# ehsan886/DBA_mod

Hardware: AMD Instinct MI355X
Metric: FL rounds/sec + backdoor ASR & main-task acc, ResNet-18 CIFAR-10 100 clients (higher is better)
Workload: dtype fp32

## Files before the change

### csrc/kernels/xconv_fwd.hip

```cpp
#include "xhalo.hpp"

namespace xg {
SplitPolicy& split_policy() {
  static SplitPolicy p;
  return p;
}
int& xstage_mode() {
  static int mode = 1;
  return mode;
}
XLast& last_launch() {
  static XLast l{};
  return l;
}
}

namespace {

template <int W, int IMGS, int BN, int WM, int WN, bool PRE>
__global__ __launch_bounds__(256) void ximg_kernel(const XArgs a) {
  constexpr int P = 2, NT = 256;
  constexpr int PW = W + 2, PI = PW * PW, PP = IMGS * PI;
  constexpr int CC = 32, CH = CC / 8, Q4 = CC / 4;
  constexpr int PATCH = PP * CH;
// ... 231 lines not shown
    split4h(pv[u].x, pv[u].y, pv[u].z, pv[u].w, hs.ma, sp);
    const int o = pp * CH + ((q >> 1) ^ (prow & 3));
#pragma unroll
    for (int p = 0; p < P; ++p) ((uint2*)&ximg2_patch[(buf * P + p) * PATCH + o])[q & 1] = sp[p];
  };

  const __amdgpu_buffer_rsrc_t rF = rsrc(a.wf + (long long)slot * a.wf_sstride, (long long)a.Ncol * 9 * Cs * 4);
  const int wbase = ((n0 >> 5) + wn) * NK * 4096 + lane * 16;
  uint4 wb[3][4];
  auto gw = [&](int t, int s, int f) __attribute__((always_inline)) {
    wb[s][f] = __builtin_bit_cast(uint4, bload4(rF, t < NK ? wbase + t * 4096 + f * 1024 : kOOB));
  };

  f32x16_t acc[MI][1];
#pragma unroll
  for (int i = 0; i < MI; ++i)
#pragma unroll
    for (int r = 0; r < 16; ++r) acc[i][0][r] = 0.f;

  int apix[MI], arow[MI];
#pragma unroll
  for (int i = 0; i < MI; ++i) {
    const int m = wm * TM + i * 32 + fr;
    const int im = m / (W * W), rem = m - im * (W * W);
    apix[i] = im * PI + (rem / W) * PW + rem % W;
    arow[i] = rem / W;
  }

  hs.init(amax_read(a.amax_src, a.amax_src_ld, g), amax_read(a.amax_w, a.amax_w_ld, slot));
#pragma unroll
  for (int f = 0; f < 4; ++f) {
    gw(0, 0, f);
    gw(1, 1, f);
  }
#pragma unroll
  for (int u = 0; u < NE; ++u) pload1(u, 0);
#pragma unroll
  for (int u = 0; u < NE; ++u) {
    ppiece(u, 0);
    pload1(u, 1);
  }
  __syncthreads();
  for (int c = 0; c < NC; ++c) {
    const uint4* L = ximg2_patch + (c & 1) * P * PATCH;
    const bool more = c + 1 < NC;
    sfor<9>([&](auto TAP) __attribute__((always_inline)) {
      constexpr int tap = decltype(TAP)::value, ti = tap / 3, tj = tap - ti * 3;
      constexpr int toff = ti * PW + tj, s = tap % 3, s2 = (tap + 2) % 3;
      constexpr int u = tap - (9 - NE);
      constexpr int NQ = u >= 0 ? 5 : 4;
      const int t = c * 9 + tap;
      __builtin_amdgcn_sched_barrier(0x786);
      sfor<2>([&](auto KK) __attribute__((always_inline)) {
        constexpr int kk = decltype(KK)::value;
        const int ch = kk * 2 + hf;
        uint4 af[P][MI], bfr[P][1];
#pragma unroll
        for (int i = 0; i < MI; ++i) {
          const int o = (apix[i] + toff) * CH + (ch ^ ((arow[i] + ti) & 3));
#pragma unroll
          for (int p = 0; p < P; ++p) af[p][i] = L[p * PATCH + o];
        }
#pragma unroll
        for (int p = 0; p < P; ++p) bfr[p][0] = wb[s][kk * 2 + p];
        mma_half<MI, 1, P, true, NQ, kk>(af, bfr, acc, [&](int q) __attribute__((always_inline)) {
          if (q < 4) {
            gw(t + 2, s2, q);
          } else if constexpr (u >= 0) {
            if (more) ppiece(u, (c + 1) & 1);
            pload1(u, c + 2);
          }
        });
      });
    });
    __syncthreads();
  }
  hs.finish(acc);

  float* out = a.out + (long long)g * a.out_gstride;
  const float* bias = a.bias ? a.bias + (long long)slot * a.b_sstride : nullptr;
  const float* res = a.res ? a.res + (long long)g * a.out_gstride : nullptr;
  float vmax = 0.f;
  const int n = n0 + wn * 32 + fr;
  if (n < a.Ncol) {
    const float bv = bias ? bias[n] : 0.f;
#pragma unroll
    for (int i = 0; i < MI; ++i)
#pragma unroll
      for (int r = 0; r < 16; ++r) {
        const int m = wm * TM + i * 32 + (r & 3) + 8 * (r >> 2) + 4 * hf;
        if (img0 + m / (W * W) >= nv) continue;
        const long long o = (long long)(img0 * W * W + m) * a.Ncol + n;
        float v = acc[i][0][r];
        if (bias) v += bv;
        if (res) v += res[o];
        if (a.relu) v = relu_nan(v);
        vmax = fmaxf(vmax, fabsf(v));
        out[o] = v;
      }
  }
  if (a.amax_out) amax_fold(a.amax_out, a.amax_out_ld, g, vmax);
}

template <int W, int IMGS, int BN, int WM, int WN>
int ximg_go(const XArgs& a, int G, hipStream_t st) {
  XArgs b = a;
  b.tiles_n = ceil_div(a.Ncol, BN);
  const dim3 grid((unsigned)(ceil_div(a.N, IMGS) * b.tiles_n), G, 1);
  xg::last_launch() = XLast{3, W, BN, a.wp != nullptr, 0, 1, 1, 0};
  if (a.wp) hipLaunchKernelGGL((ximg_kernel<W, IMGS, BN, WM, WN, true>), grid, dim3(256), 0, st, b);
  else hipLaunchKernelGGL((ximg_kernel<W, IMGS, BN, WM, WN, false>), grid, dim3(256), 0, st, b);
  DBA_LAUNCH_CHECK();
}
template <int W, int IMGS, int BN>
int ximg2_go(const XArgs& a, int G, hipStream_t st) {
  constexpr int PATCH = IMGS * (W + 2) * (W + 2) * 4;
  constexpr int LDS = 2 * 2 * PATCH * (int)sizeof(uint4);
  static unsigned long long attr_set = 0ull;
  int dev = 0;
  if (hipGetDevice(&dev) != hipSuccess || dev < 0 || dev >= 64) return -100;
  if (!(attr_set >> dev & 1ull)) {
    if (hipFuncSetAttribute((const void*)ximg2_kernel<W, IMGS, BN>, hipFuncAttributeMaxDynamicSharedMemorySize,
                            LDS) != hipSuccess)
      return -100;
    attr_set |= 1ull << dev;
  }
  XArgs b = a;
  b.tiles_n = ceil_div(a.Ncol, BN);
  const dim3 grid((unsigned)(ceil_div(a.N, IMGS) * b.tiles_n), G, 1);
  xg::last_launch() = XLast{4, W, BN, 1, 0, 1, 1, 0};
  hipLaunchKernelGGL((ximg2_kernel<W, IMGS, BN>), grid, dim3(256), LDS, st, b);
  DBA_LAUNCH_CHECK();
}
__global__ __launch_bounds__(256) void xstage16_kernel(const XArgs a) {
  constexpr int P = 2, W = 16, CS = 64, BM = 128, BN = 64, WN = 2;
  constexpr int TR = BM / W, PW = W + 2, PR = TR + 2, PP = PR * PW;
  constexpr int CH = CS / 8, PATCH = PP * CH;
  constexpr int TM = 64, TN = 32, MI = TM / 32;
  constexpr int CB = CS / 32;
  constexpr int STG = (BN / 32) * CB * 4 * 64;
  static_assert(BM * BN <= P * PATCH * 4, "epilogue tile fits the patch");
  __shared__ __attribute__((aligned(16))) uint4 lds[P * PATCH + 2 * STG];
  __shared__ long long orow[BM];
  uint4* const patch = lds;
  uint4* const bring = lds + P * PATCH;

  const int g = blockIdx.y;
  const int HT = a.Ho / TR;
  const int tm = blockIdx.x;
  const int img = tm / HT, h0 = (tm - img * HT) * TR;
  if (img >= valid_rows(a.nvalid, g, a.N)) return;
  const int slot = a.wsel ? a.wsel[g] : g;
  const float* __restrict__ src = a.src + (long long)g * a.src_gstride;
  const int tid = threadIdx.x, lane = tid & 63, wid = tid >> 6;
  const int wm = wid / WN, wn = wid % WN;
  const int fr = lane & 31, hf = lane >> 5;

  const uint16_t* F = a.wf + (long long)slot * a.wf_sstride + ((wid >> 1) * (CB * 9) + (wid & 1) * 9) * 2048 + lane * 8;
  auto fill = [&](int tap) __attribute__((always_inline)) {
    const uint32_t dst = __builtin_amdgcn_readfirstlane(
        (uint32_t)(uintptr_t)(__attribute__((address_space(3))) void*)(bring + (tap & 1) * STG + wid * 256));
#pragma unroll
    for (int f = 0; f < 4; ++f) {
      uint32_t keep;
      asm volatile("s_mov_b32 %0, m0\n\ts_mov_b32 m0, %2\n\ts_nop 0\n\tglobal_load_lds_dwordx4 %1, off\n\ts_mov_b32 m0, %0"
                   : "=&s"(keep)
                   : "v"(F + tap * 2048 + f * 512), "s"(dst + f * 1024)
                   : "memory");
    }
  };
  auto gl_sync = [&]() __attribute__((always_inline)) {
    asm volatile("s_waitcnt vmcnt(0)" ::: "memory");
    __syncthreads();
  };
  fill(0);

  if (tid < BM)
    orow[tid] = (((long long)img * a.Ho + h0 + tid / W) * a.Wo + tid % W) * a.Ncol;

  constexpr int Q4 = CS / 4;
  constexpr int NE = (PP * Q4 + 255) / 256;
  float4 pv[NE];
  {
    const __amdgpu_buffer_rsrc_t rA = rsrc(src, (long long)a.N * a.Hs * a.Ws * CS * 4);
#pragma unroll
    for (int u = 0; u < NE; ++u) {
      const int e = tid + 256 * u;
      const int pp = e / Q4, q = e - pp * Q4;
      const int pr = pp / PW, pc = pp - pr * PW;
      const int h = h0 - 1 + pr, w = pc - 1;
      const bool ok = e < PP * Q4 && (unsigned)h < (unsigned)a.Hs && (unsigned)w < (unsigned)a.Ws;
      pv[u] = bload4(rA, ok ? (((img * a.Hs + h) * a.Ws + w) * CS + q * 4) * 4 : kOOB);
    }
  }
  HScale hs;
  hs.init(amax_read(a.amax_src, a.amax_src_ld, g), amax_read(a.amax_w, a.amax_w_ld, slot));
#pragma unroll
  for (int u = 0; u < NE; ++u) {
    const int e = tid + 256 * u;
    if (e >= PP * Q4) break;
    const int pp = e / Q4, q = e - pp * Q4;
    uint2 sp[P];
    split4h(pv[u].x, pv[u].y, pv[u].z, pv[u].w, hs.ma, sp);
    const int o = pp * CH + ((q >> 1) ^ hswz<W, CS>(pp, pp % PW));
#pragma unroll
    for (int p = 0; p < P; ++p) ((uint2*)&patch[p * PATCH + o])[q & 1] = sp[p];
  }

  f32x16_t acc[MI][1];
#pragma unroll
  for (int i = 0; i < MI; ++i)
#pragma unroll
    for (int r = 0; r < 16; ++r) acc[i][0][r] = 0.f;
  int apix[MI], acol[MI];
#pragma unroll
  for (int i = 0; i < MI; ++i) {
    const int m = wm * TM + i * 32 + fr;
    apix[i] = (m / W) * PW + (m % W);
    acol[i] = m % W;
  }

  auto stage = [&](int tap) __attribute__((always_inline)) {
    const int ti = tap / 3, tj = tap - ti * 3;
    const int toff = ti * PW + tj;
    const uint4* L = bring + (tap & 1) * STG + wn * (CB * 4 * 64) + lane;
    uint4 af[2][P][MI], bfr[2][P][1];
    auto frags = [&](auto Hc) __attribute__((always_inline)) {
      constexpr int h = decltype(Hc)::value, cb = h / 2, kk = h % 2, st = h & 1;
      const int ch = kk * 2 + hf;
#pragma unroll
      for (int i = 0; i < MI; ++i) {
        const int pp = apix[i] + toff;
        const int o = pp * CH + ((cb * 4 + ch) ^ hswz<W, CS>(pp, acol[i] + tj));
#pragma unroll
        for (int p = 0; p < P; ++p) af[st][p][i] = patch[p * PATCH + o];
      }
#pragma unroll
      for (int p = 0; p < P; ++p) bfr[st][p][0] = L[(cb * 4 + kk * 2 + p) * 64];
    };
    frags(std::integral_constant<int, 0>{});
    sfor<2 * CB>([&](auto Hc) __attribute__((always_inline)) {
      constexpr int h = decltype(Hc)::value;
      if constexpr (h + 1 < 2 * CB) frags(std::integral_constant<int, h + 1>{});
      __builtin_amdgcn_sched_barrier(0);
      mma_half<MI, 1, P, true, 0, h % 2>(af[h & 1], bfr[h & 1], acc, [](int) {});
      __builtin_amdgcn_sched_barrier(0);
    });
  };

  gl_sync();
  for (int tap = 0; tap < 9; ++tap) {
    if (tap + 1 < 9) fill(tap + 1);
    stage(tap);
    gl_sync();
  }
  hs.finish(acc);

  float* Ct = reinterpret_cast<float*>(patch);
#pragma unroll
  for (int i = 0; i < MI; ++i)
#pragma unroll
    for (int r = 0; r < 16; ++r)
      Ct[(wm * TM + i * 32 + (r & 3) + 8 * (r >> 2) + 4 * hf) * BN + wn * TN + fr] = acc[i][0][r];
  __syncthreads();
  float* out = a.out + (long long)g * a.out_gstride;
  const float* bias = a.bias ? a.bias + (long long)slot * a.b_sstride : nullptr;
  const float* res = a.res ? a.res + (long long)g * a.out_gstride : nullptr;
  constexpr int C4 = BN / 4;
  float vmax = 0.f;
  for (int e = tid; e < BM * C4; e += 256) {
    const int row = e / C4, n = (e - row * C4) * 4;
    const long long o = orow[row];
    float4 v = *(const float4*)&Ct[row * BN + n];
    if (bias) { v.x += bias[n]; v.y += bias[n + 1]; v.z += bias[n + 2]; v.w += bias[n + 3]; }
    if (res) {
      const float4 rv = *(const float4*)(res + o + n);
      v.x += rv.x; v.y += rv.y; v.z += rv.z; v.w += rv.w;
    }
    if (a.relu) relu_nan4(v);
    vmax = fmaxf(vmax, fmaxf(fmaxf(fabsf(v.x), fabsf(v.y)), fmaxf(fabsf(v.z), fabsf(v.w))));
    *(float4*)(out + o + n) = v;
  }
  if (a.amax_out) amax_fold(a.amax_out, a.amax_out_ld, g, vmax);
}

constexpr bool kXStage16Default = true;

int xstage16_try(const XArgs& a, int G, int KH, int KW, hipStream_t st) {
  const XClass& c = a.cls[0];
  const int mode = xg::xstage_mode();
  if (!(mode == 3 || (mode == 1 && kXStage16Default))) return -100;
  if (KH != 3 || KW != 3 || a.sp != 1 || a.os != 1 || a.dsg != 1 || a.splitk != 1 || c.nI != 3 || c.nJ != 3 ||
      c.bh != -1 || c.bw != -1)
    return -100;
  if (a.Hs != 16 || a.Ws != 16 || a.Ho != 16 || a.Wo != 16 || a.Cs != 64 || a.Ncol != 64) return -100;
  if (a.bf.mode || a.lz_coef || a.sc_src) return -100;
  if (!aligned16(a.src) || !aligned16(a.w) || a.src_gstride % 4 || a.w_sstride % 4) return -100;
  if (!a.wp || !a.wf || ((uintptr_t)a.wf & 15) || a.wf_sstride % 8 || a.wf_sstride < 2 * 64 * 576) return -100;
  xg::last_launch() = XLast{5, 16, 64, 1, 0, 1, 1, 0};
  hipLaunchKernelGGL(xstage16_kernel, dim3((unsigned)(a.N * (a.Ho / 8)), G, 1), dim3(256), 0, st, a);
  DBA_LAUNCH_CHECK();
}

int& ximg_on() {
  static int on = 1;
  return on;
}
int ximg_try(const XArgs& a, int G, int KH, int KW, hipStream_t st) {
  const XClass& c = a.cls[0];
  if (!ximg_on() || KH != 3 || KW != 3 || a.sp != 1 || a.os != 1 || a.dsg != 1 || a.splitk != 1 || c.nI != 3 ||
      c.nJ != 3 || c.bh != -1 || c.bw != -1)
    return -100;
  if (a.Hs != a.Ho || a.Ws != a.Wo || a.Ho != a.Wo || a.Cs % 32 != 0 || a.Ncol % 32 != 0) return -100;
  if (a.bf.mode || a.lz_coef) return -100;
  if (!aligned16(a.src) || a.src_gstride % 4 || !aligned16(a.w) || a.w_sstride % 4) return -100;
  if (a.wp && (((uintptr_t)a.wp & 15) || a.wp_sstride % 8)) return -100;
  if (a.sc_src) return -100;
  if (ximg_on() == 1 && a.wp && a.wf && !((uintptr_t)a.wf & 15) && a.wf_sstride % 8 == 0) {
    int rc = -100;
    if (a.Wo == 8) rc = a.Ncol >= 128 ? ximg2_go<8, 2, 128>(a, G, st) : ximg2_go<8, 2, 64>(a, G, st);
    if (a.Wo == 4) rc = a.Ncol >= 128 ? ximg2_go<4, 8, 128>(a, G, st) : ximg2_go<4, 8, 64>(a, G, st);
    if (rc != -100) return rc;
  }
  if (a.Wo == 8) return a.Ncol >= 128 ? ximg_go<8, 2, 128, 2, 2>(a, G, st) : ximg_go<8, 2, 64, 2, 2>(a, G, st);
  if (a.Wo == 4) return a.Ncol >= 128 ? ximg_go<4, 8, 128, 2, 2>(a, G, st) : ximg_go<4, 8, 64, 2, 2>(a, G, st);
  return -100;
}

}

DBA_EXPORT int dba_xsplit_policy(int target, int min_k, int max_s, int kslab_max, int dgrad_ks) {
  SplitPolicy& p = split_policy();
  if (dgrad_ks >= 0) p.dgrad_ks = dgrad_ks;
  if (target > 0) p.target = target;
  if (min_k > 0) p.min_k = min_k;
  if (max_s > 0) p.max_s = std::min(max_s, kSkMax);
  if (kslab_max > 0) p.kslab_max = kslab_max;
  return 0;
}

DBA_EXPORT int dba_xconv_last_launch(int* out) {
  const XLast& l = xg::last_launch();
  const int v[8] = {l.kind, l.tile, l.vec, l.pre, l.form, l.slabs, l.nclass, l.lazy};
  for (int i = 0; i < 8; ++i) out[i] = v[i];
  return 0;
}

DBA_EXPORT int dba_ximg_set(int on) {
  const int prev = ximg_on();
  if (on >= 0) ximg_on() = on;
  return prev;
}

DBA_EXPORT int dba_xstage_set(int on) {
  const int prev = xg::xstage_mode();
  if (on >= 1 && on <= 3) xg::xstage_mode() = on;
  return prev;
}


DBA_EXPORT long long dba_xconv_ws_floats(int G, int N, int Ho, int Wo, int Cin, int Cout, int KH, int KW) {
  const long long M = (long long)N * Ho * Wo;
  const int s = xsplitk(M, G, Cout, KH * KW * Cin);
  return s > 1 ? (long long)s * G * M * Cout : 0;
}


DBA_EXPORT long long dba_xconv_sk_ints(int G, int N, int Ho, int Wo, int Cin, int Cout, int KH, int KW) {
  const long long M = (long long)N * Ho * Wo;
  const int s = xsplitk(M, G, Cout, KH * KW * Cin);
  const long long n = s > 1 ? xconv_sk_count(M, Cout, G, 1, s) : 0;
  return (n > 0 && sk_ok((const int*)1, n, M, Cout, G, 1, s)) ? n : 0;
}


DBA_EXPORT int dba_xconv_fwd(const float* x, long long x_gstride, const float* w, long long w_sstride,
                             const int* wsel, const float* bias, long long b_sstride, const float* res, float* out,
                             long long out_gstride, const int* nvalid, int G, int N, int H, int W, int Cin, int Ho,
                             int Wo, int Cout, int KH, int KW, int stride, int pad, int relu, const int* amax_x,
                             int amax_x_ld, const int* amax_w, int amax_w_ld, int* amax_out, int amax_out_ld,
                             const uint16_t* wp, long long wp_sstride, const uint16_t* wf, long long wf_sstride,
                             float* ws, long long ws_floats, int* sk_cnt,
                             long long sk_cnt_n, const void* bnf, const float* lz_coef, int lz_relu,
                             void* stream) {
  hipStream_t st = (hipStream_t)stream;
  if ((long long)N * H * W * Cin >= (1LL << 29)) return -103;
  const long long M = (long long)N * Ho * Wo;
  const int K = KH * KW * Cin;
  const int vec = (Cin % 4 == 0 && aligned16(x) && aligned16(w) && x_gstride % 4 == 0 && w_sstride % 4 == 0) ? 4 : 1;
  XArgs a{};
  a.src = x; a.src_gstride = x_gstride; a.w = w; a.w_sstride = w_sstride; a.wsel = wsel;
  a.bias = bias; a.b_sstride = b_sstride; a.res = res; a.out = out; a.out_gstride = out_gstride;
  a.nvalid = nvalid; a.N = N; a.Hs = H; a.Ws = W; a.Cs = Cin; a.Ncol = Cout; a.Ho = Ho; a.Wo = Wo;
  a.sp = stride; a.os = 1; a.dsg = 1; a.relu = relu; a.splitk = 1;
  a.amax_src = amax_x; a.amax_w = amax_w; a.amax_out = amax_out;
  a.amax_src_ld = amax_x_ld; a.amax_w_ld = amax_w_ld; a.amax_out_ld = amax_out_ld;
  a.wp = wp; a.wp_sstride = wp_sstride; a.wf = wf; a.wf_sstride = wf_sstride;
  a.cls[0] = XClass{KH, KW, -pad, -pad, 0, 0, Ho, Wo, 0};
  if (!amax_x || !amax_w) return -109;
  if (bnf) {
    a.bf = *(const BnFuse*)bnf;
    if (a.bf.mode != 1 || bias || res || relu || (Cout & 3) || a.bf.C != Cout) return -108;
  }
  if (lz_coef) {
    if (wp || vec < 4 || Cin > 512) return -108;
    a.lz_coef = lz_coef; a.lz_relu = lz_relu;
  }
  auto fin = [&](int rc) { return (rc == 0 && a.bf.mode) ? bnx_finalize_go(a.bf, nvalid, G, N, Ho * Wo, st) : rc; };
  if (stride == 1) {
    int rc = ximg_try(a, G, KH, KW, st);
    if (rc == -100) rc = xstage16_try(a, G, KH, KW, st);
    if (rc == -100) rc = xhalo_try(a, G, KH, KW, st);
    if (rc != -100) return fin(rc);
  }
  const int s = xsplitk(M, G, Cout, K);
  const bool ws_ok = s > 1 && ws != nullptr && ws_floats >= (long long)s * G * M * Cout;
  if (s > 1 && !(ws_ok && sk_ok(sk_cnt, sk_cnt_n, M, Cout, G, 1, s))) {
    XArgs b = a;
    b.kslab = s;
    const int rc = xconv_ks(b, M, G, vec, st);
    if (rc != -100) return fin(rc);
  }
  if (ws_ok && sk_ok(sk_cnt, sk_cnt_n, M, Cout, G, 1, s)) {
    XArgs b = a;
    b.splitk = s;
    b.zstride = (long long)G * M * Cout;
    b.sk_ws = ws; b.sk_gstride = M * Cout; b.sk_cnt = sk_cnt;
    return fin(xconv_dispatch(b, M, G, 1, vec, st));
  }
  if (ws_ok) {
    XArgs b = a;
    b.splitk = s;
    b.out = ws;
    b.out_gstride = M * Cout;
    b.zstride = (long long)G * M * Cout;
    const int rc = xconv_dispatch(b, M, G, 1, vec, st);
    if (rc != 0) return rc;
    if (a.bf.mode)
      return bnx_tile_go(a.bf, nullptr, out, out_gstride, nvalid, G, N, Ho * Wo, nullptr, 0.f, ws, s, b.zstride,
                         nullptr, st);
    const long long per = M * Cout;
    const dim3 grid((unsigned)std::max(1LL, std::min(1024LL, (per + 255) / 256)), G);
    hipLaunchKernelGGL(xsplitk_reduce_kernel, grid, dim3(256), 0, st, (const float*)ws, s, b.zstride, per, nvalid, N,
                       Ho * Wo, Cout, bias, b_sstride, wsel, res, relu, out, amax_out, amax_out_ld);
    DBA_LAUNCH_CHECK();
  }
  return fin(xconv_dispatch(a, M, G, 1, vec, st));
}


DBA_EXPORT int dba_xdown_fwd(const float* a_, long long a_gstride, const float* w2, long long w2_sstride,
                             const uint16_t* w2p, long long w2p_sstride, const int* wsel, const float* b2,
                             long long b_sstride, const float* x2, long long x2_gstride, const uint16_t* wscp,
                             long long wscp_sstride, const float* bsc, long long bsc_sstride, float* out,
                             long long out_gstride, const int* nvalid, int G, int N, int Ho, int Wo, int C, int H2,
                             int W2, int C2, const int* amax_a, int amax_a_ld, const int* amax_w2, int amax_w2_ld,
                             const int* amax_x2, int amax_x2_ld, const int* amax_wsc, int amax_wsc_ld, int* amax_out,
                             int amax_out_ld, void* stream) {
  if (!amax_a || !amax_w2 || !amax_x2 || !amax_wsc || !w2p || !wscp) return -109;
  if ((H2 - 1) / 2 + 1 != Ho || (W2 - 1) / 2 + 1 != Wo || (long long)N * H2 * W2 * C2 >= (1LL << 29) ||
      (long long)N * Ho * Wo * C >= (1LL << 29))
    return -103;
  XArgs a{};
  a.src = a_; a.src_gstride = a_gstride; a.w = w2; a.w_sstride = w2_sstride; a.wsel = wsel;
  a.bias = b2; a.b_sstride = b_sstride; a.res = nullptr; a.out = out; a.out_gstride = out_gstride;
  a.nvalid = nvalid; a.N = N; a.Hs = Ho; a.Ws = Wo; a.Cs = C; a.Ncol = C; a.Ho = Ho; a.Wo = Wo;
  a.sp = 1; a.os = 1; a.dsg = 1; a.relu = 1; a.splitk = 1;
  a.amax_src = amax_a; a.amax_w = amax_w2; a.amax_out = amax_out;
  a.amax_src_ld = amax_a_ld; a.amax_w_ld = amax_w2_ld; a.amax_out_ld = amax_out_ld;
  a.wp = w2p; a.wp_sstride = w2p_sstride;
  a.sc_src = x2; a.sc_gstride = x2_gstride; a.sc_H = H2; a.sc_W = W2; a.sc_C = C2;
  a.sc_wp = wscp; a.sc_wp_sstride = wscp_sstride;
  a.sc_amax_src = amax_x2; a.sc_amax_src_ld = amax_x2_ld; a.sc_amax_w = amax_wsc; a.sc_amax_w_ld = amax_wsc_ld;
  a.sc_bias = bsc; a.sc_b_sstride = bsc_sstride;
  a.cls[0] = XClass{3, 3, -1, -1, 0, 0, Ho, Wo, 0};
  return xhalo_try(a, G, 3, 3, (hipStream_t)stream);
}
```

### dba_mod_amd/ops/hip.py

```python
from __future__ import annotations

import contextlib
import ctypes
import os
from typing import Optional, Sequence, Tuple

import torch

from . import bnstate as bs
from . import build
from . import reference as _ref

Tensor = torch.Tensor
_F32 = torch.float32

if not os.path.exists(build.kernels_path()):
    raise ImportError(f"HIP kernel library missing: {build.kernels_path()} — run "
                      f"`python -m dba_mod_amd.ops.build` (or __graft_entry__.build())")
_L = ctypes.CDLL(build.kernels_path())

_P = ctypes.c_void_p
_I = ctypes.c_int
_LL = ctypes.c_longlong
_F = ctypes.c_float
_U = ctypes.c_uint
_D = ctypes.c_double

_SIGS = {
    "dba_gather_images": [_P, _P, _P, _P, _P, _P, _I, _P, _P, _I, _P, _I, _I, _I, _I, _I, _P],
    "dba_gather_rows": [_P, _P, _P, _P, _P, _I, _P, _P, _I, _P, _I, _P, _I, _I, _I, _P],
    "dba_xcolsum": [_P, _LL, _I, _P, _I, _I, _I, _P, _LL, _P, _P],
    "dba_xcolsum_part_doubles": [_I, _I, _I, _I],
    "dba_amax_segments": [_P, _LL, _P, _I, _I, _P, _I, _P],
    "dba_bn_fold": [_P, _LL, _P, _P, _P, _P, _P, _LL, _F, _P, _P, _I, _I, _I, _I, _P, _I, _P],
    "dba_relu_mask_bwd": [_P, _P, _P, _LL, _I, _P],
    "dba_maxpool": [_P, _P, _P, _LL, _I, _I, _I, _I, _I, _I, _I, _I, _I, _P],
    "dba_maxpool_bwd": [_P, _P, _P, _LL, _I, _I, _I, _I, _I, _I, _I, _I, _I, _P],
    "dba_avgpool": [_P, _P, _LL, _I, _I, _I, _P],
    "dba_avgpool_bwd": [_P, _P, _LL, _I, _I, _I, _P],
    "dba_dropout": [_P, _P, _I, _P, _U, _F, _LL, _I, _P],
    "dba_softmax_xent": [_P, _P, _I, _I, _I, _I, _P, _P, _P, _P, _LL, _P, _I, _P, _I, _P, _P, _P],
    "dba_softmax_xent_part_doubles": [_I, _I],
    "dba_xent_r5_set": [_I],
    "dba_head_train": [_P, _LL, _I, _I, _I, _I, _P, _LL, _P, _LL, _I, _P, _P, _P, _P, _P, _P, _LL, _P, _LL, _P, _P,
                       _P, _P, _LL, _P, _I, _I, _P],
    "dba_head_part_doubles": [_I, _I],
    "dba_sgd_step": [_P, _LL, _P, _P, _P, _P, _P, _F, _F, _P, _I, _I, _P],
    "dba_scale_from_base": [_P, _P, _F, _P, _LL, _P],
    "dba_add_noise_scaled": [_P, _P, _LL, _F, _F, _U, _I, _I, _P],
    "dba_delta_sum": [_P, _LL, _I, _P, _LL, _P, _P],
    "dba_sqdist_blocks": [_LL],
    "dba_gram_chunks": [_I],
    "dba_sq_dists": [_P, _LL, _P, _I, _LL, _P, _P, _P],
    "dba_weighted_sum": [_P, _LL, _P, _I, _P, _LL, _I, _P],
    "dba_weighted_sum_fixed": [_P, _LL, _P, _I, _P, _LL, _D, _P],
    "dba_gram": [_P, _LL, _I, _I, _P, _P, _P],
    "dba_delta_stats_blocks": [_LL],
    "dba_delta_stats": [_P, _LL, _I, _P, _LL, _P, _P, _P, _P, _P],
    "dba_clipped_delta_sum_fixed": [_P, _LL, _I, _P, _P, _P, _LL, _D, _P],
    "dba_clipped_delta_sum": [_P, _LL, _I, _P, _P, _P, _LL, _P],
    "dba_pairwise_sqdist_blocks": [_LL],
    "dba_pairwise_sqdist": [_P, _LL, _P, _I, _LL, _P, _P, _P],
    "dba_delta_gram_blocks": [_LL],
    "dba_delta_gram": [_P, _LL, _P, _I, _P, _LL, _P, _P, _P],
    "dba_coord_trim_blocks": [_LL],
    "dba_coord_trim": [_P, _LL, _P, _I, _P, _I, _LL, _P, _P, _P, _P],
    "dba_coord_bulyan_blocks": [_LL],
    "dba_coord_bulyan": [_P, _LL, _P, _I, _P, _I, _LL, _P, _P, _P, _P],
    "dba_vote_agreement_blocks": [_LL],
    "dba_rlr_apply_blocks": [_LL],
    "dba_delta_sum_votes": [_P, _LL, _I, _P, _LL, _P, _P, _P],
    "dba_vote_agreement": [_P, _LL, _I, _P, _P, _I, _LL, _P, _P, _P],
    "dba_rlr_apply": [_P, _P, _P, _I, _LL, _F, _F, _U, _I, _P, _P, _P],
    "dba_topk_select_blocks": [_LL],
    "dba_topk_apply_blocks": [_LL],
    "dba_topk_ws_words": [],
    "dba_topk_select": [_P, _P, _LL, _LL, _P, _P, _P],
    "dba_topk_apply": [_P, _P, _P, _LL, _F, _P, _P],
    "dba_dist_loss_grad": [_P, _LL, _P, _LL, _P, _LL, _I, _P, _P, _F, _P, _P, _P],
    "dba_project_to_ball": [_P, _LL, _P, _LL, _LL, _I, _P, _P, _D, _P, _P, _P, _P],
    "dba_nmask_blocks": [_LL],
    "dba_nmask_block_sweep": [],
    "dba_nmask_blocks_max": [],
    "dba_nmask_ws_words": [],
    "dba_neurotoxin_mask": [_P, _P, _LL, _LL, _P, _P, _P, _P],
    "dba_mask_restore": [_P, _LL, _P, _LL, _LL, _I, _P, _P, _P, _P, _P],
    "dba_ximg_set": [_I],
    "dba_xwgrad_halo_set": [_I],
    "dba_xconv_ws_floats": [_I] * 8,
    "dba_xconv_fwd": [_P, _LL, _P, _LL, _P, _P, _LL, _P, _P, _LL, _P] + [_I] * 13 + [_P, _I] * 3 + [_P, _LL] * 3
    + [_P, _LL, _P, _P, _I, _P],
    "dba_xconv_sk_ints": [_I] * 8,
    "dba_xconv_dgrad": [_P, _LL, _P, _LL, _P, _P, _P, _LL, _P] + [_I] * 12 + [_P, _I] * 2 + [_P, _LL] * 3 + [_P, _P],
    "dba_xsplit_w": [_P, _LL, _LL, _I, _P, _I, _P, _P],
    "dba_amax": [_P, _LL, _LL, _P, _LL, _I, _P, _I, _P],
    "dba_xtranspose": [_P, _I, _I, _LL, _P, _P],
    "dba_xwgrad_ws_floats": [_I] * 8 + [_P],
    "dba_xwgrad_stem_ws_floats": [_I] * 6,
    "dba_xsplit_policy": [_I] * 5,
    "dba_xsplit_w_batch": [_P, _I, _I, _P],
    "dba_xfrag_w_batch": [_P, _I, _I, _P],
    "dba_bn_fold_batch": [_P, _I, _I, _F, _P],
    "dba_xwgrad": [_P, _LL, _P, _LL, _P, _LL, _P] + [_I] * 12 + [_P, _I] * 2 + [_P, _LL, _I] + [_P, _I, _P],
    "dba_bnx_rows": [_P, _P, _P, _LL, _P, _I, _I, _I, _P, _F, _P],
    "dba_bnx_apply": [_P, _P, _P, _P, _P, _I, _I, _P, _LL, _P, _I, _I, _I, _I, _P, _I, _P],
    "dba_bnfuse_size": [],
    "dba_xwgrad_stem": [_P, _LL, _P, _P, _P, _LL, _P, _P, _I, _I, _I, _I, _P],
    "dba_bnx_dy": [_P, _P, _P, _P, _LL, _P, _I, _I, _I, _I, _P, _I, _P],
    "dba_xwgrad_reduce_batch": [_P, _I, _I, _LL, _P],
    "dba_xstage_set": [_I],
    "dba_xblock_fwd": [_P, _LL, _P, _LL, _P, _P, _P, _LL, _P, _P, _LL, _P, _P, _LL, _P] + [_I] * 6
    + [_P, _I, _P, _P, _I, _P, _I, _P],
    "dba_xblock_stem_fwd": [_P, _LL, _P, _LL, _P, _P, _LL, _P, _LL, _P, _P, _LL, _P, _P, _LL, _P, _P, _LL, _P]
    + [_I] * 6 + [_P, _P, _P, _I, _P, _I, _P],
    "dba_mlp_train": [_P, _I, _I, _I, _I, _I, _P, _LL, _P, _P, _I, _P, _I, _I, _I, _I, _P, _P, _P, _P, _I, _I,
                      _P, _LL, _I, _P, _F, _F, _P, _P],
    "dba_xdown_fwd": [_P, _LL, _P, _LL, _P, _LL, _P, _P, _LL, _P, _LL, _P, _LL, _P, _LL, _P, _LL, _P] + [_I] * 8
    + [_P, _I] * 5 + [_P],
    "dba_xconv_last_launch": [_P],
    "dba_xstem_fwd": [_P, _LL, _P, _LL, _P, _P, _LL, _P, _P, _LL, _P] + [_I] * 13 + [_P, _I, _P, _P],
}
for _name, _args in _SIGS.items():
    _fn = getattr(_L, _name)
    _fn.argtypes = _args
    _fn.restype = ctypes.c_int
_L.dba_xconv_ws_floats.restype = ctypes.c_longlong
_L.dba_xconv_sk_ints.restype = ctypes.c_longlong
_L.dba_xwgrad_ws_floats.restype = ctypes.c_longlong
_L.dba_xwgrad_stem_ws_floats.restype = ctypes.c_longlong
_L.dba_xcolsum_part_doubles.restype = ctypes.c_longlong
_L.dba_softmax_xent_part_doubles.restype = ctypes.c_longlong
_L.dba_head_part_doubles.restype = ctypes.c_longlong


class _BnFuse(ctypes.Structure):
    _fields_ = [("mode", _I), ("C", _I), ("ngrp", _I),
                ("rec0", _P),
                ("coef_a", _P), ("gamma_a", _P), ("beta_a", _P), ("rm_a", _P), ("rv_a", _P),
                ("p_gstride", _LL), ("momentum", _F), ("eps", _F), ("relu", _I),
                ("amax_a", _P), ("amax_ld", _I),
                ("ya", _P), ("yb", _P), ("y_gstride", _LL),
                ("coef_b", _P), ("gamma_b", _P), ("amax_b", _P),
                ("dgamma_a", _P), ("dbeta_a", _P), ("dgamma_b", _P), ("dbeta_b", _P), ("gr_gstride", _LL),
                ("mask_out", _P), ("mask_lazy", _I)]


assert ctypes.sizeof(_BnFuse) == int(_L.dba_bnfuse_size()), "BnFuse layout mismatch (rebuild the kernels)"


NOT_HANDLED = -100
F16_PAIR = 16


def _call(name: str, *args) -> int:
    rc = getattr(_L, name)(*args)
    if rc != 0 and rc != NOT_HANDLED:
        raise RuntimeError(f"{name}: HIP error {rc}")
    return rc


def _ptr(t: Optional[Tensor]):
    return None if t is None else t.data_ptr()


def _stream():
    return torch.cuda.current_stream().cuda_stream


def _i32(t: Optional[Tensor]) -> Optional[Tensor]:
    if t is None:
        return None
    return t if (t.dtype == torch.int32 and t.is_contiguous()) else t.to(torch.int32).contiguous()


def _inner_contig(t: Tensor) -> bool:
    exp = 1
    for d in range(t.dim() - 1, 0, -1):
        if t.shape[d] != 1 and t.stride(d) != exp:
            return False
        exp *= t.shape[d]
    return True


def _rowview(t: Tensor) -> Tuple[Tensor, int]:
    if not _inner_contig(t):
        t = t.contiguous()
    return t, (t.stride(0) if t.shape[0] > 1 else int(torch.tensor(t.shape[1:]).prod()))


def _act(t: Tensor, dt: Optional[torch.dtype] = None, what: str = "activation") -> Tensor:
    if t.dtype != _F32:
        raise TypeError(f"{what}: unsupported dtype {t.dtype} (fp32 only)")
    if dt is not None and t.dtype != dt:
        raise TypeError(f"{what}: dtype {t.dtype} does not match the op's {dt} operands "
                        f"(no silent precision conversion)")
    return t.contiguous()


def _f32(t: Tensor) -> int:
    return int(t.dtype == _F32)


_UNIT_AMAX = {}


def _unit_amax(G: int, device):
    key = (G, device)
    if key not in _UNIT_AMAX:
        a = torch.zeros(AMAX_SUB, _amax_ld(G), dtype=torch.int32, device=device)
        a[0, :G] = 0x3F800000
        _UNIT_AMAX[key] = a
    return _UNIT_AMAX[key]


def gather_images(src, labels, idx, trig_masks, trig_id, poison_n, target, flip_seeds, out_dtype):
    G, B = idx.shape
    _, H, W, C = src.shape
    x = torch.empty(G, B, H, W, C, dtype=out_dtype, device=src.device)
    y = torch.empty(G, B, dtype=torch.int32, device=src.device)
    idx, trig_id, poison_n, fs = _i32(idx), _i32(trig_id), _i32(poison_n), _i32(flip_seeds)
    _call("dba_gather_images", src.data_ptr(), _i32(labels).data_ptr(), idx.data_ptr(),
          trig_masks.contiguous().data_ptr(), trig_id.data_ptr(), poison_n.data_ptr(), int(target), _ptr(fs),
          x.data_ptr(), int(out_dtype == torch.float32), y.data_ptr(), G, B, H, W, C, _stream())
    if out_dtype == _F32:
        x._dba_amax = _unit_amax(G, x.device)
    return x, y


def gather_rows(src, labels, idx, trig_cols, trig_vals, trig_id, poison_n, target, out_dtype):
    G, B = idx.shape
    Fd = src.shape[1]
    x = torch.empty(G, B, Fd, dtype=out_dtype, device=src.device)
    y = torch.empty(G, B, dtype=torch.int32, device=src.device)
    tc = _i32(trig_cols)
    _call("dba_gather_rows", src.contiguous().data_ptr(), _i32(labels).data_ptr(), _i32(idx).data_ptr(),
          tc.data_ptr(), trig_vals.float().contiguous().data_ptr(), int(tc.shape[1]), _i32(trig_id).data_ptr(),
          _i32(poison_n).data_ptr(), int(target), x.data_ptr(), int(out_dtype == torch.float32), y.data_ptr(),
          G, B, Fd, _stream())
    return x, y


_MLP_LAYERS = ("layer1.0.weight", "layer1.0.bias", "layer2.0.weight", "layer2.0.bias", "layer3.0.weight",
               "layer3.0.bias")


def mlp_train(spec, sched, t0, t1, B, state, mom, fg, rows, labels, trig_cols, trig_vals, target, stats,
              max_slots, nan_flag, momentum, wd, prof=None) -> int:
    G = state.shape[0]
    es = [spec.by_name[n] for n in _MLP_LAYERS]
    offs = torch.tensor([e.offset for e in es], dtype=torch.int32)
    (H1, F), (H2, _), (C, _) = es[0].k_shape[:2], es[2].k_shape[:2], es[4].k_shape[:2]
    assert sched.dtype == torch.int32 and sched.is_contiguous() and state.stride(1) == 1
    tc = _i32(trig_cols)
    return _call("dba_mlp_train", sched.data_ptr(), sched.shape[1], int(t0), int(t1), G, B, state.data_ptr(),
                 state.stride(0), mom.data_ptr(), _ptr(fg), spec.P, offs.data_ptr(), F, H1, H2, C,
                 rows.contiguous().data_ptr(), _i32(labels).data_ptr(), tc.data_ptr(),
                 trig_vals.float().contiguous().data_ptr(), int(tc.shape[1]), int(target), stats.data_ptr(),
                 stats.shape[1], max_slots, nan_flag.data_ptr(), float(momentum), float(wd), _ptr(prof), _stream())


def _check_w(w: Tensor, dt: torch.dtype = _F32) -> Tuple[Tensor, int]:
    if w.dtype != dt:
        raise TypeError(f"conv weights: dtype {w.dtype} does not match the {dt} activations "
                        f"(no silent precision conversion)")
    return _rowview(w)


def last_conv_launch() -> dict:
    a = (ctypes.c_int * 8)()
    _L.dba_xconv_last_launch(ctypes.cast(a, ctypes.c_void_p))
    return dict(zip(("kind", "tile", "vec", "pre", "form", "slabs", "nclass", "lazy"), (int(v) for v in a)))


def set_ximg(on: int) -> int:
    return int(_L.dba_ximg_set(int(on)))


def set_xstage(on: int) -> int:
    return int(_L.dba_xstage_set(int(on)))


def set_wgrad_halo(on: int) -> int:
    return int(_L.dba_xwgrad_halo_set(int(on)))


def set_split_policy(target: int = -1, min_k: int = -1, max_s: int = -1, kslab_max: int = -1,
                     dgrad_ks: int = -1) -> None:
    _call("dba_xsplit_policy", int(target), int(min_k), int(max_s), int(kslab_max), int(dgrad_ks))


_STEM_WGRAD = True


def set_stem_wgrad(on: int) -> int:
    global _STEM_WGRAD
    prev = int(_STEM_WGRAD)
    if on >= 0:
        _STEM_WGRAD = bool(on)
    return prev


def fp32_mode() -> int:
    return F16_PAIR


AMAX_SUB = 16


def _amax_ld(G: int) -> int:
    return max(32, (G + 31) // 32 * 32)


class _AmaxArena:

    def __init__(self, G: int, device, n: int, counters: int = 0) -> None:
        self.G, self.ld, self.next = G, _amax_ld(G), 0
        slots = n * AMAX_SUB * self.ld
        flat = torch.zeros(slots + counters, dtype=torch.int32, device=device)
        self.buf = flat[:slots].view(n, AMAX_SUB, self.ld)
        self.cnt, self.cnt_next = flat[slots:], 0

    def counters(self, n: int, device):
        if n <= 0 or device != self.cnt.device or self.cnt_next + n > self.cnt.numel():
            return None
        self.cnt_next += n
        return self.cnt[self.cnt_next - n:self.cnt_next]

    def take(self, G: int, device):
        if G != self.G or self.next >= self.buf.shape[0] or device != self.buf.device:
            return None
        self.next += 1
        return self.buf[self.next - 1]


_ARENA: list = []


@contextlib.contextmanager
def amax_arena(G: int, device, n: int = 256, counters: int = 0):
    _ARENA.append(_AmaxArena(G, device, n, counters))
    try:
        yield
    finally:
        _ARENA.pop()


def amax_slots(n: int, G: int, device):
    return torch.zeros(n, AMAX_SUB, _amax_ld(G), dtype=torch.int32, device=device)


def _amax_new(G: int, device):
    a = _ARENA[-1].take(G, device) if _ARENA else None
    return a if a is not None else torch.zeros(AMAX_SUB, _amax_ld(G), dtype=torch.int32, device=device)


def _sk_counters(n: int, device):
    if n <= 0 or not _ARENA:
        return None
    return _ARENA[-1].counters(n, device)


def _aptr(a):
    return (None, 0) if a is None else (a.data_ptr(), a.shape[-1])


def _amax(t, gstride, n_per_g, nvalid=None, per_item=0):
    G = t.shape[0]
    out = _amax_new(G, t.device)
    _call("dba_amax", t.data_ptr(), gstride, n_per_g, _ptr(_i32(nvalid)), per_item, G, out.data_ptr(), out.shape[1],
          _stream())
    return out


def _amax_out(t):
    if t.dtype != _F32:
        return None
    a = _amax_new(t.shape[0], t.device)
    t._dba_amax = a
    return a


def weight_amax(flat, segments):
    G, n = flat.shape[0], len(segments)
    ar = _ARENA[-1] if _ARENA else None
    if ar is not None and ar.G == G and ar.buf.device == flat.device and ar.next + n <= ar.buf.shape[0]:
        buf, ar.next = ar.buf[ar.next:ar.next + n], ar.next + n
    else:
        buf = torch.zeros(n, AMAX_SUB, _amax_ld(G), dtype=torch.int32, device=flat.device)
    slots, base = list(buf), buf.data_ptr()
    d = torch.tensor(segments, dtype=torch.int64)
    _call("dba_amax_segments", flat.data_ptr(), flat.stride(0), d.data_ptr(), len(segments), G, base,
          slots[0].shape[1], _stream())
    return slots


def split_weights(w, sstride: int, per: int, amax):
    slots = w.shape[0]
    out = torch.empty(slots, 2, per, dtype=torch.int16, device=w.device)
    _call("dba_xsplit_w", w.data_ptr(), sstride, per, slots, amax.data_ptr(), amax.shape[1], out.data_ptr(), _stream())
    w._dba_planes = out
    frag_weights_batch([w])
    return out


def split_weights_batch(items) -> None:
    if not items:
        return
    slots = items[0][0].shape[0]
    desc, outs = [], []
    for w, sstride, per, amax in items:
        assert w.shape[0] == slots and w.dtype == torch.float32
        out = torch.empty(slots, 2, per, dtype=torch.int16, device=w.device)
        desc.append([w.data_ptr(), sstride, per, amax.data_ptr(), amax.shape[1], out.data_ptr(), 0])
        outs.append(out)
    d = torch.tensor(desc, dtype=torch.int64)
    _call("dba_xsplit_w_batch", d.data_ptr(), len(items), slots, _stream())
    for (w, *_), out in zip(items, outs):
        w._dba_planes = out
    frag_weights_batch([w for w, *_ in items])


def frag_weights_batch(ws) -> None:
    desc, outs = [], []
    for w in ws:
        p = getattr(w, "_dba_planes", None)
        if (p is None or w.dim() != 5 or tuple(w.shape[2:4]) != (3, 3) or w.shape[1] % 32 or w.shape[4] % 32
                or not p.is_contiguous() or p.shape[2] != w[0].numel()):
            continue
        out = torch.empty(p.shape[0], 2 * p.shape[2], dtype=torch.int16, device=p.device)
        desc.append([p.data_ptr(), out.data_ptr(), w.shape[1], w.shape[4], 0])
        outs.append((w, out))
    if not desc:
        return
    d = torch.tensor(desc, dtype=torch.int64)
    _call("dba_xfrag_w_batch", d.data_ptr(), len(desc), outs[0][1].shape[0], _stream())
    for w, out in outs:
        w._dba_fplanes = out


def _wplanes(w):
    p = getattr(w, "_dba_planes", None)
    return (None, 0) if p is None else (p.data_ptr(), p.stride(0))


def _wfplanes(w):
    p = getattr(w, "_dba_fplanes", None)
    return (None, 0) if p is None else (p.data_ptr(), p.stride(0))


def _wfplanes2(w1, w2):
    (f1, s1), (f2, s2) = _wfplanes(w1), _wfplanes(w2)
    return (f1, f2, s1) if f1 is not None and f2 is not None and s1 == s2 else (None, None, 0)


def _amax_w(w, gstride, n):
    a = getattr(w, "_dba_amax", None)
    if a is None:
        a = _amax(w, gstride, n)
        w._dba_amax = a
    return a


def _amax_act(t, nvalid):
    a = getattr(t, "_dba_amax", None)
    if a is not None:
        return a
    per_item = t[0, 0].numel()
    a = _amax(t, t.stride(0), t.shape[1] * per_item, nvalid, per_item)
    t._dba_amax = a
    return a


_EVAL_STEM_MFMA = os.environ.get("DBA_EVAL_STEM7_MFMA", "1") != "0"
_EVAL_STEM_PAD = True


def _xconv_fwd(x, w, wsel, stride, pad, bias, residual, relu, nvalid, out_dtype, bnf=None, lz=None):
    if out_dtype not in (None, _F32):
        raise TypeError(f"fp32 conv cannot emit {out_dtype} (no silent precision conversion)")
    G, N, H, W, Cin = x.shape
    attrs = {k: getattr(w, k) for k in ("_dba_amax", "_dba_planes", "_dba_fplanes") if hasattr(w, k)}
    w, ws = _check_w(w, _F32)
    for k, v in attrs.items():
        setattr(w, k, v)
    Cout, KH, KW = w.shape[1], w.shape[2], w.shape[3]
    assert w.shape[4] == Cin, (w.shape, x.shape)
    Ho = (H + 2 * pad - KH) // stride + 1
    Wo = (W + 2 * pad - KW) // stride + 1
    y = torch.empty(G, N, Ho, Wo, Cout, dtype=_F32, device=x.device)
    bs = 0
    if bias is not None:
        if bias.dtype != _F32:
            raise TypeError(f"conv bias must be fp32 (got {bias.dtype})")
        bias, bs = _rowview(bias)
    res = _act(residual, _F32, "residual") if residual is not None else None
    ay = _amax_out(y) if bnf is None else None
    bnf_p = ctypes.byref(bnf) if bnf is not None else None
    eval_mfma = (_EVAL_STEM_MFMA and "_dba_planes" in attrs and bnf is None and KH * KW * Cin > 64)
    if eval_mfma and Cin % 4 and _EVAL_STEM_PAD and lz is None:
        cp = 4 - Cin % 4
        x4 = torch.nn.functional.pad(x, (0, cp))
        x4._dba_amax = _amax_act(x, nvalid)
        w4 = torch.nn.functional.pad(w, (0, cp)).contiguous()
        per4 = w4[0].numel()
        a4 = attrs.get("_dba_amax")
        split_weights(w4, per4, per4, a4 if a4 is not None else _amax_w(w4, per4, per4))
        if a4 is not None:
            w4._dba_amax = a4
        return _xconv_fwd(x4, w4, wsel, stride, pad, bias, residual, relu, nvalid, out_dtype)
    if Cin <= 4 and not eval_mfma:
        rc = _call("dba_xstem_fwd", x.data_ptr(), N * H * W * Cin, w.data_ptr(), ws, _ptr(_i32(wsel)), _ptr(bias), bs,
                   _ptr(res), y.data_ptr(), N * Ho * Wo * Cout, _ptr(_i32(nvalid)), G, N, H, W, Cin, Ho, Wo, Cout,
                   KH, KW, stride, pad, int(relu), *_aptr(ay), bnf_p, _stream())
        if rc != NOT_HANDLED:
            return y
    n = int(_L.dba_xconv_ws_floats(G, N, Ho, Wo, Cin, Cout, KH, KW))
    wsb = torch.empty(n, dtype=_F32, device=x.device) if n > 0 else None
    ncnt = int(_L.dba_xconv_sk_ints(G, N, Ho, Wo, Cin, Cout, KH, KW)) if n > 0 else 0
    cnt = _sk_counters(ncnt, x.device)
    ax = lz[2] if lz is not None else _amax_act(x, nvalid)
    aw = _amax_w(w, ws, Cout * KH * KW * Cin)
    lz_coef, lz_relu = (lz[0].data_ptr(), int(lz[1])) if lz is not None else (None, 0)
    _call("dba_xconv_fwd", x.data_ptr(), N * H * W * Cin, w.data_ptr(), ws, _ptr(_i32(wsel)), _ptr(bias), bs,
          _ptr(res), y.data_ptr(), N * Ho * Wo * Cout, _ptr(_i32(nvalid)), G, N, H, W, Cin, Ho, Wo, Cout, KH, KW,
          stride, pad, int(relu), *_aptr(ax), *_aptr(aw), *_aptr(ay), *_wplanes(w), *_wfplanes(w), _ptr(wsb), n,
          _ptr(cnt), 0 if cnt is None else cnt.numel(), bnf_p, lz_coef, lz_relu, _stream())
    return y


_EVAL_BLOCK = os.environ.get("DBA_EVAL_BLOCK", "1") != "0"
_BLOCK_SHAPES = {(32, 32)}


def basic_block_ok(x, w1, w2) -> bool:
    if not (_EVAL_BLOCK and x.dtype == _F32 and x.dim() == 5):
        return False
    H, W, C = x.shape[2:]
    return (H == W and (W, C) in _BLOCK_SHAPES
            and all(w.dtype == _F32 and tuple(w.shape[1:]) == (C, 3, 3, C)
                    and getattr(w, "_dba_planes", None) is not None for w in (w1, w2)))


def basic_block_eval(x, w1, b1, w2, b2, wsel=None, nvalid=None):
    x = _act(x, _F32, "conv input")
    G, N, _, W, C = x.shape
    per = C * 9 * C
    (w1c, ws1), (w2c, ws2) = _check_w(w1), _check_w(w2)
    aw1, aw2 = _amax_w(w1, ws1, per), _amax_w(w2, ws2, per)
    p1, p2 = w1._dba_planes, w2._dba_planes
    assert p1.stride(0) == p2.stride(0) and aw1.shape[1] == aw2.shape[1]
    (b1c, bs1), (b2c, bs2) = _rowview(b1), _rowview(b2)
    assert bs1 == bs2 and b1c.dtype == b2c.dtype == _F32
    ax = _amax_act(x, nvalid)
    y = torch.empty_like(x)
    ay = _amax_out(y)
    rc = _call("dba_xblock_fwd", x.data_ptr(), x.stride(0), y.data_ptr(), y.stride(0), _ptr(_i32(wsel)),
               p1.data_ptr(), p2.data_ptr(), p1.stride(0), *_wfplanes2(w1, w2), b1c.data_ptr(), b2c.data_ptr(), bs1,
               _ptr(_i32(nvalid)), G, N, W, W, C, C, *_aptr(ax), aw1.data_ptr(), aw2.data_ptr(), aw1.shape[1], *_aptr(ay), _stream())
    if rc == NOT_HANDLED:
        raise RuntimeError("xblock_fwd declined a shape basic_block_ok accepted")
    return y


_EVAL_STEM = os.environ.get("DBA_EVAL_STEM", "1") != "0"


def stem_block_ok(x, w0, w1, w2) -> bool:
    if not (_EVAL_STEM and _EVAL_BLOCK and x.dtype == _F32 and x.dim() == 5 and tuple(x.shape[2:]) == (32, 32, 3)):
        return False
    return (w0.dtype == _F32 and tuple(w0.shape[1:]) == (32, 3, 3, 3) and getattr(w0, "_dba_planes", None) is not None
            and all(w.dtype == _F32 and tuple(w.shape[1:]) == (32, 3, 3, 32)
                    and getattr(w, "_dba_planes", None) is not None for w in (w1, w2)))


def stem_block_eval(x, w0, b0, w1, b1, w2, b2, wsel=None, nvalid=None):
    x = _act(x, _F32, "image")
    G, N, _, W, Ci = x.shape
    C = w1.shape[1]
    per = C * 9 * C
    (w0c, ws0), (w1c, ws1), (w2c, ws2) = _check_w(w0), _check_w(w1), _check_w(w2)
    aw0 = _amax_w(w0, ws0, C * 9 * Ci)
    aw1, aw2 = _amax_w(w1, ws1, per), _amax_w(w2, ws2, per)
# ... 881 lines not shown
```

Before: 3.855.

## Add dedicated stride-2 3x3 conv forward kernel with phase-split swizzled LDS patch

Adds a specialized HIP kernel for the stride-2 3x3 conv with 32x32x32 input and 16x16x64 output. It stages the input patch in LDS split into four row/column parity planes with an XOR swizzle to avoid bank conflicts, keeps weights in registers, and double-buffers patch loads across persistent tiles. It replaces the generic split-K or implicit-GEMM path for this layer shape. The cost is dynamic LDS sizing and a narrowly gated fast path.

Result: no change. 3.883, median of 6 (+0.7%).

```diff
diff --git a/csrc/kernels/xconv_fwd.hip b/csrc/kernels/xconv_fwd.hip
--- a/csrc/kernels/xconv_fwd.hip
+++ b/csrc/kernels/xconv_fwd.hip
@@ -557,6 +557,174 @@
   DBA_LAUNCH_CHECK();
 }
 
+struct XS2 {
+  static constexpr int P = 2, TR = 4, WO = 16, HS = 32, CS = 32, BN = 64, BM = TR * WO;
+  static constexpr int SW0 = 17, SW1 = 16, SR0 = TR + 1, SR1 = TR;
+  static constexpr int O00 = 0, O01 = O00 + SR0 * SW0, O10 = O01 + SR0 * SW1, O11 = O10 + SR1 * SW0;
+  static constexpr int PP = O11 + SR1 * SW1;
+  static constexpr int CH = 4, PATCH = PP * CH;
+  static constexpr int LDS = 2 * P * PATCH * (int)sizeof(uint4);
+  static constexpr int TPB = 16;
+  static_assert(PP == (2 * TR + 1) * 33, "patch");
+};
+__global__ __launch_bounds__(256, 2) void xs2_kernel(const XArgs a) {
+  using X = XS2;
+  constexpr int P = X::P, TR = X::TR, WO = X::WO, HS = X::HS, CS = X::CS, BN = X::BN, BM = X::BM;
+  constexpr int CH = X::CH, PATCH = X::PATCH, HT = WO / TR;
+  extern __shared__ __attribute__((aligned(16))) uint4 xs2_patch[];
+
+  const int g = blockIdx.y;
+  const int nt = min(valid_rows(a.nvalid, g, a.N), a.N) * HT;
+  const int t0 = blockIdx.x * X::TPB, t1 = min(t0 + X::TPB, nt);
+  if (t0 >= nt) return;
+  const int slot = a.wsel ? a.wsel[g] : g;
+  const float* __restrict__ src = a.src + (long long)g * a.src_gstride;
+  const int tid = threadIdx.x, lane = tid & 63, wid = tid >> 6;
+  const int wm = wid >> 1, wn = wid & 1;
+  const int fr = lane & 31, hf = lane >> 5;
+
+  uint4 wb[9][4];
+  {
+    const __amdgpu_buffer_rsrc_t rF = rsrc(a.wf + (long long)slot * a.wf_sstride, (long long)BN * 9 * CS * 4);
+    const int wbase = wn * 9 * 4096 + lane * 16;
+#pragma unroll
+    for (int t = 0; t < 9; ++t)
+#pragma unroll
+      for (int f = 0; f < 4; ++f) wb[t][f] = __builtin_bit_cast(uint4, bload4(rF, wbase + t * 4096 + f * 1024));
+  }
+
+  auto opaque = [](int v) __attribute__((always_inline)) {
+    asm volatile("" : "+v"(v));
+    return v;
+  };
+  constexpr int Q4 = CS / 4;
+  constexpr int NE = (X::PP * Q4 + 255) / 256;
+  float4 pv[NE];
+  const __amdgpu_buffer_rsrc_t rA = rsrc(src, (long long)a.N * HS * HS * CS * 4);
+  auto pload = [&](int t) __attribute__((always_inline)) {
+    const int img = t / HT, h0 = (t - img * HT) * TR;
+    const int tl = opaque(tid);
+#pragma unroll
+    for (int u = 0; u < NE; ++u) {
+      const int e = tl + 256 * u;
+      const int pp = e / Q4, q = e - pp * Q4;
+      const int pr = pp / 33, pc = pp - pr * 33;
+      const int h = 2 * h0 - 1 + pr, w = pc - 1;
+      const bool ok = e < X::PP * Q4 && (unsigned)h < (unsigned)HS && (unsigned)w < (unsigned)HS;
+      pv[u] = bload4(rA, ok ? (((img * HS + h) * HS + w) * CS + q * 4) * 4 : kOOB);
+    }
+  };
+  HScale hs;
+  auto pstore = [&](int buf) __attribute__((always_inline)) {
+    uint4* const patch = xs2_patch + buf * P * PATCH;
+    const int tl = opaque(tid);
+#pragma unroll
+    for (int u = 0; u < NE; ++u) {
+      const int e = tl + 256 * u;
+      if (e >= X::PP * Q4) break;
+      const int pp = e / Q4, q = e - pp * Q4;
+      const int pr = pp / 33, pc = pp - pr * 33;
+      const int sr = pr >> 1, sc = pc >> 1;
+      const int pix = (pc & 1) ? ((pr & 1) ? X::O11 : X::O01) + sr * X::SW1 + sc
+                               : ((pr & 1) ? X::O10 : X::O00) + sr * X::SW0 + sc;
+      const int key = (pc & 1) ? (sc >> 2) & 3 : (((sc + sr) >> 1) + sr) & 3;
+      uint2 sp[P];
+      split4h(pv[u].x, pv[u].y, pv[u].z, pv[u].w, hs.ma, sp);
+      const int o = pix * CH + ((q >> 1) ^ key);
+#pragma unroll
+      for (int p = 0; p < P; ++p) ((uint2*)&patch[p * PATCH + o])[q & 1] = sp[p];
+    }
+  };
+
+  const int m = wm * 32 + fr, aoh = m / WO, aow = m % WO;
+  const int ap0 = aoh * X::SW0 + aow, ap1 = aoh * X::SW1 + aow;
+
+  float* const out = a.out + (long long)g * a.out_gstride;
+  const int n = wn * 32 + fr;
+  const float bv = a.bias ? a.bias[(long long)slot * a.b_sstride + n] : 0.f;
+  float vmax = 0.f;
+
+  pload(t0);
+  hs.init(amax_read(a.amax_src, a.amax_src_ld, g), amax_read(a.amax_w, a.amax_w_ld, slot));
+  pstore(0);
+  __syncthreads();
+  for (int t = t0, buf = 0; t < t1; ++t, buf ^= 1) {
+    const bool more = t + 1 < t1;
+    if (more) pload(t + 1);
+    const uint4* const patch = xs2_patch + buf * P * PATCH;
+    f32x16_t acc[1][1];
+#pragma unroll
+    for (int r = 0; r < 16; ++r) acc[0][0][r] = 0.f;
+
+    uint4 af[2][P][1], bfr[2][P][1];
+    auto frags = [&](auto Hc) __attribute__((always_inline)) {
+      constexpr int h = decltype(Hc)::value, tap = h / 2, kk = h % 2, st = h & 1;
+      constexpr int ti = tap / 3, tj = tap - ti * 3, dI = ti == 2, dJ = tj == 2;
+      constexpr int SW = (tj & 1) ? X::SW1 : X::SW0;
+      constexpr int base = ((tj & 1) ? ((ti & 1) ? X::O11 : X::O01) : ((ti & 1) ? X::O10 : X::O00)) + dI * SW + dJ;
+      const int pix = base + ((tj & 1) ? ap1 : ap0);
+      const int key = (tj & 1) ? (aow >> 2) & 3 : (((aow + aoh + dI + dJ) >> 1) + aoh + dI) & 3;
+      const int o = pix * CH + ((kk * 2 + hf) ^ key);
+#pragma unroll
+      for (int p = 0; p < P; ++p) {
+        af[st][p][0] = patch[p * PATCH + o];
+        bfr[st][p][0] = wb[tap][kk * 2 + p];
+      }
+    };
+    frags(std::integral_constant<int, 0>{});
+    sfor<18>([&](auto Hc) __attribute__((always_inline)) {
+      constexpr int h = decltype(Hc)::value;
+      if constexpr (h + 1 < 18) frags(std::integral_constant<int, h + 1>{});
+      __builtin_amdgcn_sched_barrier(0);
+      mma_half<1, 1, P, true, 0, h % 2>(af[h & 1], bfr[h & 1], acc, [](int) {});
+      __builtin_amdgcn_sched_barrier(0);
+    });
+    hs.finish(acc);
+    if (more) pstore(buf ^ 1);
+
+    float* const ot = out + (long long)t * (BM * BN) + n;
+#pragma unroll
+    for (int r = 0; r < 16; ++r) {
+      float v = acc[0][0][r];
+      if (a.bias) v += bv;
+      if (a.relu) v = relu_nan(v);
+      vmax = fmaxf(vmax, fabsf(v));
+      ot[(wm * 32 + (r & 3) + 8 * (r >> 2) + 4 * hf) * BN] = v;
+    }
+    __syncthreads();
+  }
+  if (a.amax_out) amax_fold(a.amax_out, a.amax_out_ld, g, vmax);
+}
+
+int& xs2_mode() {
+  static int mode = 1;
+  return mode;
+}
+int xs2_try(const XArgs& a, int G, int KH, int KW, hipStream_t st) {
+  const XClass& c = a.cls[0];
+  if (!xs2_mode()) return -100;
+  if (KH != 3 || KW != 3 || a.sp != 2 || a.os != 1 || a.dsg != 1 || a.splitk != 1 || c.nI != 3 || c.nJ != 3 ||
+      c.bh != -1 || c.bw != -1)
+    return -100;
+  if (a.Hs != 32 || a.Ws != 32 || a.Ho != 16 || a.Wo != 16 || a.Cs != 32 || a.Ncol != 64) return -100;
+  if (a.bf.mode || a.lz_coef || a.sc_src || a.res) return -100;
+  if (!aligned16(a.src) || a.src_gstride % 4) return -100;
+  if (!a.wp || !a.wf || ((uintptr_t)a.wf & 15) || a.wf_sstride % 8 || a.wf_sstride < 2 * 64 * 288) return -100;
+  static unsigned long long attr_set = 0ull;
+  int dev = 0;
+  if (hipGetDevice(&dev) != hipSuccess || dev < 0 || dev >= 64) return -100;
+  if (!(attr_set >> dev & 1ull)) {
+    if (hipFuncSetAttribute((const void*)xs2_kernel, hipFuncAttributeMaxDynamicSharedMemorySize, XS2::LDS) != hipSuccess)
+      return -100;
+    attr_set |= 1ull << dev;
+  }
+  xg::last_launch() = XLast{10, 16, 64, 1, 0, 1, 1, 0};
+  const dim3 grid((unsigned)ceil_div((long long)a.N * (XS2::WO / XS2::TR), XS2::TPB), G, 1);
+  hipLaunchKernelGGL(xs2_kernel, grid, dim3(256), XS2::LDS, st, a);
+  DBA_LAUNCH_CHECK();
+}
+
+
 int& ximg_on() {
   static int on = 1;
   return on;
@@ -610,6 +778,12 @@
 DBA_EXPORT int dba_xstage_set(int on) {
   const int prev = xg::xstage_mode();
   if (on >= 1 && on <= 3) xg::xstage_mode() = on;
+  return prev;
+}
+
+DBA_EXPORT int dba_xs2_set(int on) {
+  const int prev = xs2_mode();
+  if (on == 0 || on == 1) xs2_mode() = on;
   return prev;
 }
 
@@ -669,6 +843,10 @@
     if (rc != -100) return fin(rc);
   }
   const int s = xsplitk(M, G, Cout, K);
+  if (stride == 2 && s == 1) {
+    const int rc = xs2_try(a, G, KH, KW, st);
+    if (rc != -100) return fin(rc);
+  }
   const bool ws_ok = s > 1 && ws != nullptr && ws_floats >= (long long)s * G * M * Cout;
   if (s > 1 && !(ws_ok && sk_ok(sk_cnt, sk_cnt_n, M, Cout, G, 1, s))) {
     XArgs b = a;
diff --git a/dba_mod_amd/ops/hip.py b/dba_mod_amd/ops/hip.py
--- a/dba_mod_amd/ops/hip.py
+++ b/dba_mod_amd/ops/hip.py
@@ -109,6 +109,7 @@
     "dba_bnx_dy": [_P, _P, _P, _P, _LL, _P, _I, _I, _I, _I, _P, _I, _P],
     "dba_xwgrad_reduce_batch": [_P, _I, _I, _LL, _P],
     "dba_xstage_set": [_I],
+    "dba_xs2_set": [_I],
     "dba_xblock_fwd": [_P, _LL, _P, _LL, _P, _P, _P, _LL, _P, _P, _LL, _P, _P, _LL, _P] + [_I] * 6
     + [_P, _I, _P, _P, _I, _P, _I, _P],
     "dba_xblock_stem_fwd": [_P, _LL, _P, _LL, _P, _P, _LL, _P, _LL, _P, _P, _LL, _P, _P, _LL, _P, _P, _LL, _P]
@@ -278,6 +279,10 @@
 
 def set_xstage(on: int) -> int:
     return int(_L.dba_xstage_set(int(on)))
+
+
+def set_xs2(on: int) -> int:
+    return int(_L.dba_xs2_set(int(on)))
 
 
 def set_wgrad_halo(on: int) -> int:
diff --git a/profiles/r9/xs2/swizzle_enum.py b/profiles/r9/xs2/swizzle_enum.py
--- /dev/null
+++ b/profiles/r9/xs2/swizzle_enum.py
@@ -0,0 +1,36 @@
+from collections import Counter
+
+GROUPS = [list(range(0, 4)) + list(range(12, 16)) + list(range(20, 28)),
+          list(range(4, 12)) + list(range(16, 20)) + list(range(28, 32))]
+TR = 4
+SW = [17, 16]
+SR = [TR + 1, TR]
+
+
+def extra(key):
+    off, o = {}, 0
+    for rp in (0, 1):
+        for cp in (0, 1):
+            off[rp, cp] = o
+            o += SR[rp] * SW[cp]
+    groups = bad = tot = 0
+    for ti in range(3):
+        for tj in range(3):
+            rp, cp = ti & 1, tj & 1
+            for base in range(0, TR * 16, 32):
+                for ch in range(4):
+                    for g in GROUPS:
+                        slots = []
+                        for fr in g:
+                            m = base + fr
+                            sr, sc = m // 16 + (ti == 2), m % 16 + (tj == 2)
+                            pix = off[rp, cp] + sr * SW[cp] + sc
+                            slots.append((pix * 4 + (ch ^ key(pix, sr, sc, cp))) % 16)
+                        c = sum(n - 1 for n in Counter(slots).values())
+                        groups, bad, tot = groups + 1, bad + (c > 0), tot + c
+    return groups, bad, tot
+
+
+print("(pixel >> 2) & 3            : groups %d, conflicting %d, extra lanes %d" % extra(lambda p, sr, sc, cp: (p >> 2) & 3))
+print("xs2_kernel's keys           : groups %d, conflicting %d, extra lanes %d"
+      % extra(lambda p, sr, sc, cp: (sc >> 2) & 3 if cp else (((sc + sr) >> 1) + sr) & 3))
```
